# nmwsharp/diffusion-net

Hardware: NVIDIA H100
Metric: DiffusionNetBlock forward Mverts/sec at V=200k,K=128,C=128; 1/2/4/8 GPU (higher is better)
Workload: dtype f32

## Files before the change

### diffusion-net_b200/csrc/dn_tc.cu

```cuda
#include "dn_internal.h"
#include "dn_tc_ptx.cuh"
#include <cuda.h>
#include <cudaTypedefs.h>
#include <cuda_bf16.h>
#include <string.h>

namespace {

using namespace tc;

constexpr int KC = 16;
constexpr int TILE_M = 128;
constexpr int W_RING_BYTES = 128 * 1024;
constexpr int W_NST_MAX = 8;
constexpr int CHAIN_THREADS = 384;
constexpr int A_BOX_BYTES = 8 * TILE_M * 4;
constexpr int A_STAGE_BYTES = 2 * A_BOX_BYTES;
constexpr int A_NST_MAX = 8;
constexpr int SMEM_OPTIN = 232448;
constexpr int OUT_ROWS = 64;
constexpr int OUT_BOX_BYTES = 8 * OUT_ROWS * 4;

template <int MODE, int NMAX>
struct ChainRing {
  static constexpr int STAGE = KC * NMAX * (MODE == MODE_TF32X3 ? 8 : MODE == MODE_TF32 ? 4 : 2);
  static constexpr int NST_FULL = W_RING_BYTES / STAGE < W_NST_MAX ? W_RING_BYTES / STAGE : W_NST_MAX;
  static constexpr int STG = NMAX <= 128 && MODE != MODE_BF16 ? 2 * OUT_ROWS * NMAX * 4 : 0;
  static constexpr int BIAS = (NMAX <= 128 ? DN_MAX_LAYERS : 1) * NMAX * 4;
  static constexpr int bars(int nst, int anst) { return 8 * (2 * nst + 2 * anst + 2); }
  static constexpr int bytes(int nst, int anst) { return nst * STAGE + anst * A_STAGE_BYTES + STG + BIAS + bars(nst, anst); }
  static constexpr bool kFull = bytes(NST_FULL, A_NST_MAX) <= SMEM_OPTIN;
  static constexpr int NST = kFull ? NST_FULL : NST_FULL - 2;
  static constexpr int A_NST = kFull ? A_NST_MAX : A_NST_MAX - 1;
  static constexpr int BARS = bars(NST, A_NST);
  static constexpr int SMEM = bytes(NST, A_NST);
  static_assert(SMEM <= SMEM_OPTIN, "rows_chain_kernel: shared memory over the opt-in limit");
};

__host__ __device__ __forceinline__ int64_t stage_stride(int N) { return (int64_t)KC * N * 8; }
__host__ __device__ __forceinline__ int64_t packed_bytes(int K, int N) {
  return (((K + KC - 1) / KC) * stage_stride(N) + 255) / 256 * 256;
}

struct PackJob {
  const float* W;
  const float* W2;
  float* dst;
  int64_t ldw;
  int n_split, w_trans, K, N, blk0, fmt;
};
constexpr int kMaxPackJobs = 3 + DN_MAX_LAYERS;
struct PackJobs {
  PackJob j[kMaxPackJobs];
  int n;
  TcSpectral sp;
  int sp_blocks;
  int64_t sp_stride;
};

__device__ __forceinline__ void pack_store(float* dst, int fmt, int N, int k, int n, float w) {
  char* base = reinterpret_cast<char*>(dst) + (int64_t)(k / KC) * stage_stride(N);
  const int kk = k % KC;
  if (fmt == 2) {
    *reinterpret_cast<__nv_bfloat16*>(base + kmajor_off<MODE_BF16>(kk, n, N)) = __float2bfloat16_rn(w);
    return;
  }
  float hi, lo;
  split_tf32(w, hi, lo);
  char* q = base + kmajor_off<MODE_TF32>(tf32_k_slot(kk), n, N);
  *reinterpret_cast<float*>(q) = hi;
  *reinterpret_cast<float*>(q + (int64_t)KC * N * 4) = lo;
}

__global__ void pack_weights_kernel(const __grid_constant__ PackJobs jobs) {
  int n, k;
  float w;
  if (jobs.sp.partial && (int)blockIdx.x < jobs.sp_blocks * jobs.sp.n_meshes) {
    const PackJob& J = jobs.j[0];
    const int K = J.K, N = J.N;
    __shared__ float red[8][33];
    const int b = jobs.sp.n_meshes > 1 ? (int)blockIdx.x / jobs.sp_blocks : 0;
    const int e = threadIdx.x & 31, sl = threadIdx.x >> 5;
    const int idx = ((int)blockIdx.x - b * jobs.sp_blocks) * 32 + e;
    if (jobs.sp.plain) {
      if (sl != 0 || idx >= K * N) return;
      pack_store(J.dst + b * jobs.sp_stride, J.fmt, N, idx / N, idx % N, jobs.sp.partial[(int64_t)b * K * N + idx]);
      return;
    }
    const int p0 = jobs.sp.mesh_cta_begin ? jobs.sp.mesh_cta_begin[b] : 0;
// ... 10 lines not shown
    k = idx / N; n = idx % N;
    const float sum = pairwise_sum<8>(&red[0][e], 33);
    const float t = dn_clamp_time(jobs.sp.time[n]);
    w = dn_heat(jobs.sp.evals[(int64_t)b * K + k], t) * sum;
    pack_store(J.dst + b * jobs.sp_stride, J.fmt, N, k, n, w);
    if (jobs.sp.sum_out) jobs.sp.sum_out[(int64_t)b * K * N + idx] = sum;
    if (b == 0 && k == K - 1 && !jobs.sp.no_clamp_writeback) jobs.sp.time[n] = t;
    return;
  }
  int ji = 0;
#pragma unroll
  for (int i = 1; i < kMaxPackJobs; ++i)
    if (i < jobs.n && (int)blockIdx.x >= jobs.j[i].blk0) ji = i;
  const PackJob& J = jobs.j[ji];
  const int K = J.K, N = J.N;
  const int idx = ((int)blockIdx.x - J.blk0) * blockDim.x + threadIdx.x;
  if (idx >= K * N) return;
  n = idx / K; k = idx % K;
  if (J.w_trans) w = (J.W2 && k >= J.n_split) ? J.W2[(int64_t)(k - J.n_split) * J.ldw + n] : J.W[(int64_t)k * J.ldw + n];
  else if (J.W2 && n >= J.n_split) w = J.W2[(int64_t)(n - J.n_split) * J.ldw + k];
  else w = J.W[(int64_t)n * J.ldw + k];
  pack_store(J.dst, J.fmt, N, k, n, w);
}

struct HcLayer {
  const float* wpack;
  const float* bias;
  const float* emul;
  const float* relu_mask;
  const float* row_scale;
  const float* residual;
  int64_t ld_res;
  float res_scale;
  float* out;
  int64_t ld_out;
  int K, N, relu, sibling;
};

struct HcParams {
  CUtensorMap amap[DN_MAX_SRC];
  CUtensorMap omap[DN_MAX_LAYERS];
  CUtensorMap rmap[DN_MAX_LAYERS];
  DnRowsSrc src;
  HcLayer layer[DN_MAX_LAYERS];
  int n_layers;
  int64_t V;
  const int32_t* tile_group;
  int64_t group_stride;
  const float* head_w;
  const float* head_b;
  float* head_out;
  int64_t ld_head_out;
  int head_n;
};
static_assert(sizeof(HcParams) <= 4096, "HcParams must fit the 4 KiB kernel parameter space");

template <int MODE, int NMAX, bool WIDE>
__global__ void __launch_bounds__(CHAIN_THREADS, 1) rows_chain_kernel(const __grid_constant__ HcParams p) {
  constexpr bool kChain = NMAX <= 128;
  constexpr bool kStage = ChainRing<MODE, NMAX>::STG > 0;
  constexpr int NB = NMAX / 16;
  using Ring = ChainRing<MODE, NMAX>;
  constexpr int NST = Ring::NST, STAGE_BYTES = Ring::STAGE, A_NST = Ring::A_NST;
  extern __shared__ __align__(1024) uint8_t smem[];
  uint8_t* aring = smem + NST * STAGE_BYTES;
  uint8_t* stage_out = aring + A_NST * A_STAGE_BYTES;
  float* sbias = reinterpret_cast<float*>(stage_out + Ring::STG);
  uint64_t* bars = reinterpret_cast<uint64_t*>(stage_out + Ring::STG + Ring::BIAS);
  const uint32_t full = smem_u32(bars), empty = smem_u32(bars + NST);
  const uint32_t afull = smem_u32(bars + 2 * NST), aempty = smem_u32(bars + 2 * NST + A_NST);
  const uint32_t rfull = smem_u32(bars + 2 * NST + 2 * A_NST);
  const int warp = threadIdx.x >> 5, lane = threadIdx.x & 31;
  if (threadIdx.x == 0) {
    for (int i = 0; i < NST; ++i) { mbar_init(full + 8 * i, 1); mbar_init(empty + 8 * i, 8); }
    for (int i = 0; i < A_NST; ++i) { mbar_init(afull + 8 * i, 1); mbar_init(aempty + 8 * i, 8); }
    for (int i = 0; i < 2; ++i) mbar_init(rfull + 8 * i, 1);
    fence_barrier_init();
  }
  __syncthreads();
  const int L = p.n_layers;
  const int64_t ntiles = (p.V + TILE_M - 1) / TILE_M;

  if (warp >= 8) {
    setmaxnreg_dec<40>();
    if (warp == 9 && lane == 0) {
      const int K0 = p.layer[0].K, nst0 = (K0 + KC - 1) / KC;
      uint32_t s = 0, ph = 0;
      for (int64_t tile = blockIdx.x; tile < ntiles; tile += gridDim.x)
        for (int c = 0; c < nst0; ++c) {
          const int nbox = c * KC + 8 < K0 ? 2 : 1;
          mbar_wait(aempty + 8 * s, ph ^ 1);
          mbar_arrive_expect_tx(afull + 8 * s, (uint32_t)(nbox * A_BOX_BYTES));
          for (int h = 0; h < nbox; ++h) {
            int kc = c * KC + 8 * h, sidx = 0;
            while (sidx + 1 < p.src.nsrc && kc >= p.src.width[sidx]) { kc -= p.src.width[sidx]; ++sidx; }
            tma_tile_2d_g2s(smem_u32(aring + s * A_STAGE_BYTES + h * A_BOX_BYTES), &p.amap[sidx], kc,
                            (int)(tile * TILE_M), afull + 8 * s);
          }
          if (++s == A_NST) { s = 0; ph ^= 1; }
        }
    }
    if (warp == 8 && lane == 0) {
      uint32_t s = 0, ph = 0;
      for (int64_t tile = blockIdx.x; tile < ntiles; tile += gridDim.x)
        for (int l = 0; l < L; ++l) {
          const HcLayer& Lr = p.layer[l];
          const int nst = (Lr.K + KC - 1) / KC;
          const int64_t sstride = stage_stride(Lr.N);
          const uint32_t bytes = (uint32_t)(MODE == MODE_TF32X3 ? sstride : (MODE == MODE_TF32 ? sstride / 2 : sstride / 4));
          const char* w = reinterpret_cast<const char*>(Lr.wpack);
          if (l == 0 && p.tile_group) w += (int64_t)__ldg(p.tile_group + tile) * p.group_stride * 4;
          for (int c = 0; c < nst; ++c) {
            mbar_wait(empty + 8 * s, ph ^ 1);
            mbar_arrive_expect_tx(full + 8 * s, bytes);
            tma_bulk_g2s(smem_u32(smem + s * STAGE_BYTES), w + c * sstride, bytes, full + 8 * s);
            if (++s == NST) { s = 0; ph ^= 1; }
          }
        }
    }
    return;
  }

  setmaxnreg_inc<232>();
  for (int l = 0; l < L; ++l) {
    const HcLayer& Lr = p.layer[l];
    if (!Lr.bias) continue;
    for (int n = threadIdx.x; n < Lr.N; n += 256) sbias[l * NMAX + n] = __ldg(Lr.bias + n);
  }
  named_bar_sync(1, 256);
  const int g = lane >> 2, t = lane & 3;
  const int rloc = (warp >> 2) * 64 + (warp & 3) * 16 + g;
  const int wg = warp >> 2;
  const bool elected = (threadIdx.x & 127) == 0;
  auto stg_box = [&](int b) { return reinterpret_cast<float*>(stage_out) + (wg * NMAX + 8 * b) * OUT_ROWS; };
  float acc[NB * 8];
  float act[kChain ? NB * 8 : 1];
  uint32_t s = 0, ph = 0, as = 0, aph = 0, rph = 0;

  for (int64_t tile = blockIdx.x; tile < ntiles; tile += gridDim.x) {
    const int64_t r0 = tile * TILE_M + rloc, r1 = r0 + 8;
    const bool ok0 = r0 < p.V, ok1 = r1 < p.V;
    const int row0 = (int)(tile * TILE_M) + wg * OUT_ROWS;
    for (int l = 0; l < L; ++l) {
      const HcLayer& Lr = p.layer[l];
      const int N = WIDE ? NMAX : Lr.N, nb = N / 16;
      const int K = (WIDE && l > 0) ? NMAX : Lr.K, nst = (K + KC - 1) / KC;
      const uint32_t lbo = (uint32_t)N * 16;
      int prev = -1;
      if constexpr (kStage) {
        if (Lr.residual && elected) {
          bulk_wait_read<0>();
          if (row0 < p.V) {
            mbar_arrive_expect_tx(rfull + 8 * wg, (uint32_t)(Lr.N / 8 * OUT_BOX_BYTES));
            for (int b = 0; b < Lr.N / 8; ++b)
              tma_tile_2d_g2s(smem_u32(stg_box(b)), &p.rmap[l], 8 * b, row0, rfull + 8 * wg);
          } else {
            mbar_arrive(rfull + 8 * wg);
          }
        }
      }
      auto prefetch_rows = [&](const float* base, int64_t ld) {
#pragma unroll
        for (int h = 0; h < 2; ++h) {
          if (!(h ? ok1 : ok0)) continue;
          const char* row = reinterpret_cast<const char*>(base + (h ? r1 : r0) * ld);
          for (int b = 128 * t; b < N * 4; b += 512) prefetch_l2(row + b);
          if (t == 0) prefetch_l2(row + N * 4 - 4);
        }
      };
      if (!kStage && Lr.residual) prefetch_rows(Lr.residual, Lr.ld_res);
      if (Lr.emul) prefetch_rows(Lr.emul, N);
      if (Lr.relu_mask) prefetch_rows(Lr.relu_mask, N);
      auto stage = [&](int c, const float2* q, bool two) {
        mbar_wait(full + 8 * s, ph);
        constexpr int SLICES = MODE == MODE_BF16 ? 1 : 2;
        uint32_t ah[2][4], al[2][4];
        if constexpr (MODE == MODE_BF16) {
          const float x[8] = {q[0].x, q[0].y, q[1].x, q[1].y, q[2].x, q[2].y, q[3].x, q[3].y};
          frag_bf16(x, ah[0]);
        } else {
#pragma unroll
          for (int ks = 0; ks < 2; ++ks) {
            const float2 u = q[2 * ks], v = q[2 * ks + 1];
            const float x[4] = {u.x, v.x, u.y, v.y};
            frag_tf32(x, ah[ks], al[ks]);
          }
        }
        const uint32_t sb = smem_u32(smem + s * STAGE_BYTES);
        wgmma_fence();
#pragma unroll
        for (int ks = 0; ks < SLICES; ++ks) {
          if (ks == 1 && !two) break;
          const uint32_t acc0 = (c > 0 || ks > 0) ? 1u : 0u;
          const uint32_t base = sb + ks * 2 * lbo;
          if constexpr (WIDE) {
            mma_step<MODE, NMAX>(acc, ah[ks], al[ks], base, KC * N * 4, lbo, acc0);
          } else {
#pragma unroll
            for (int j = 0; j < NB; ++j) {
              if (j >= nb) break;
              mma_step<MODE, 16>(acc + 8 * j, ah[ks], al[ks], base + j * 256, KC * N * 4, lbo, acc0);
            }
          }
        }
        wgmma_commit();
        if constexpr (WIDE && MODE != MODE_BF16) {
          wgmma_wait<0>();
          if (lane == 0) mbar_arrive(empty + 8 * s);
        } else {
          wgmma_wait<1>();
          if (prev >= 0 && lane == 0) mbar_arrive(empty + 8 * prev);
          prev = (int)s;
        }
        if (++s == NST) { s = 0; ph ^= 1; }
      };

      if (l == 0) {
        for (int c = 0; c < nst; ++c) {
          const bool two = c * KC + 8 < K;
          mbar_wait(afull + 8 * as, aph);
          const float* a = reinterpret_cast<const float*>(aring + as * A_STAGE_BYTES) + rloc * 8 + 2 * t;
          float2 q[4];
          q[0] = *reinterpret_cast<const float2*>(a);
          q[1] = *reinterpret_cast<const float2*>(a + 64);
          q[2] = q[3] = make_float2(0.f, 0.f);
          if (two) {
            q[2] = *reinterpret_cast<const float2*>(a + A_BOX_BYTES / 4);
            q[3] = *reinterpret_cast<const float2*>(a + A_BOX_BYTES / 4 + 64);
          }
          stage(c, q, two);
          fence_proxy_async();
          __syncwarp();
          if (lane == 0) mbar_arrive(aempty + 8 * as);
          if (++as == A_NST) { as = 0; aph ^= 1; }
        }
      } else if constexpr (kChain) {
#pragma unroll
        for (int c = 0; c < NB; ++c) {
          if (c >= nst) break;
          const float2 q[4] = {make_float2(act[8 * c], act[8 * c + 1]), make_float2(act[8 * c + 2], act[8 * c + 3]),
                               make_float2(act[8 * c + 4], act[8 * c + 5]), make_float2(act[8 * c + 6], act[8 * c + 7])};
          stage(c, q, WIDE || c * KC + 8 < K);
        }
      }
      wgmma_wait<0>();
#pragma unroll
      for (int j = 0; j < NB; ++j) fence_acc8(acc + 8 * j);
      if (prev >= 0 && lane == 0) mbar_arrive(empty + 8 * prev);

      const bool last = l + 1 == L;
      const bool head = last && p.head_w != nullptr;
      const bool keep_act = !last && p.layer[l + 1].sibling;
      const float rs0 = (Lr.row_scale && ok0) ? __ldg(Lr.row_scale + r0) : 1.f;
      const float rs1 = (Lr.row_scale && ok1) ? __ldg(Lr.row_scale + r1) : 1.f;
      float hp0[kChain ? 1 : 8], hp1[kChain ? 1 : 8];
#pragma unroll
      for (int o = 0; o < (kChain ? 1 : 8); ++o) hp0[o] = hp1[o] = 0.f;
      if constexpr (kStage) {
        if (Lr.residual) {
          if (elected) mbar_wait(rfull + 8 * wg, rph);
          rph ^= 1;
          named_bar_sync(2 + wg, 128);
        } else if (Lr.out) {
          if (elected) bulk_wait_read<0>();
          named_bar_sync(2 + wg, 128);
        }
      }
      const int nb_epi = Lr.N / 16;
#pragma unroll
      for (int j = 0; j < NB; ++j) {
        if (j >= nb_epi) break;
#pragma unroll
        for (int h = 0; h < 2; ++h) {
          const int col = 16 * j + 8 * h + 2 * t;
          float* d = acc + 8 * j + 4 * h;
          float2 v0 = make_float2(d[0], d[1]), v1 = make_float2(d[2], d[3]);
          if (Lr.bias) {
            const float2 b = *reinterpret_cast<const float2*>(sbias + l * NMAX + col);
            const float b0 = b.x, b1 = b.y;
            v0.x += b0; v0.y += b1; v1.x += b0; v1.y += b1;
          }
          if (Lr.relu) {
            v0.x = fmaxf(v0.x, 0.f); v0.y = fmaxf(v0.y, 0.f); v1.x = fmaxf(v1.x, 0.f); v1.y = fmaxf(v1.y, 0.f);
          }
          if (Lr.emul) {
            if (ok0) { const float2 e = __ldg(reinterpret_cast<const float2*>(Lr.emul + r0 * N + col)); v0.x *= e.x; v0.y *= e.y; }
            if (ok1) { const float2 e = __ldg(reinterpret_cast<const float2*>(Lr.emul + r1 * N + col)); v1.x *= e.x; v1.y *= e.y; }
          }
          if (Lr.relu_mask) {
            if (ok0) {
              const float2 m = __ldg(reinterpret_cast<const float2*>(Lr.relu_mask + r0 * N + col));
              v0.x = m.x > 0.f ? v0.x : 0.f; v0.y = m.y > 0.f ? v0.y : 0.f;
            }
            if (ok1) {
              const float2 m = __ldg(reinterpret_cast<const float2*>(Lr.relu_mask + r1 * N + col));
              v1.x = m.x > 0.f ? v1.x : 0.f; v1.y = m.y > 0.f ? v1.y : 0.f;
            }
          }
          if (Lr.row_scale) { v0.x *= rs0; v0.y *= rs0; v1.x *= rs1; v1.y *= rs1; }
          if constexpr (kStage) {
            float* so = stg_box(2 * j + h) + ((warp & 3) * 16 + g) * 8 + 2 * t;
            if (Lr.residual) {
              const float2 ra = *reinterpret_cast<const float2*>(so), rb = *reinterpret_cast<const float2*>(so + 64);
              v0.x = fmaf(Lr.res_scale, ra.x, v0.x); v0.y = fmaf(Lr.res_scale, ra.y, v0.y);
              v1.x = fmaf(Lr.res_scale, rb.x, v1.x); v1.y = fmaf(Lr.res_scale, rb.y, v1.y);
            }
            if (Lr.out) {
              *reinterpret_cast<float2*>(so) = v0;
              *reinterpret_cast<float2*>(so + 64) = v1;
            }
          } else {
            if (Lr.residual) {
              if (ok0) {
                const float2 r = __ldg(reinterpret_cast<const float2*>(Lr.residual + r0 * Lr.ld_res + col));
                v0.x = fmaf(Lr.res_scale, r.x, v0.x); v0.y = fmaf(Lr.res_scale, r.y, v0.y);
              }
              if (ok1) {
                const float2 r = __ldg(reinterpret_cast<const float2*>(Lr.residual + r1 * Lr.ld_res + col));
                v1.x = fmaf(Lr.res_scale, r.x, v1.x); v1.y = fmaf(Lr.res_scale, r.y, v1.y);
              }
            }
            if (Lr.out) {
              if (ok0) *reinterpret_cast<float2*>(Lr.out + r0 * Lr.ld_out + col) = v0;
              if (ok1) *reinterpret_cast<float2*>(Lr.out + r1 * Lr.ld_out + col) = v1;
            }
          }
          if constexpr (kChain) {
            if (!keep_act) {
              act[8 * j + 4 * h] = v0.x; act[8 * j + 4 * h + 1] = v0.y;
              act[8 * j + 4 * h + 2] = v1.x; act[8 * j + 4 * h + 3] = v1.y;
            }
          }
          if (!kChain && head) {
#pragma unroll
            for (int o = 0; o < (kChain ? 1 : 8); ++o) {
              if (o >= p.head_n) break;
              const float2 w = __ldg(reinterpret_cast<const float2*>(p.head_w + (int64_t)o * N + col));
              hp0[o] = fmaf(w.y, v0.y, fmaf(w.x, v0.x, hp0[o]));
              hp1[o] = fmaf(w.y, v1.y, fmaf(w.x, v1.x, hp1[o]));
            }
          }
        }
      }
      if constexpr (kStage) {
        if (Lr.out || Lr.residual) {
          fence_proxy_async();
          named_bar_sync(2 + wg, 128);
          if (Lr.out && elected && row0 < p.V) {
            for (int b = 0; b < Lr.N / 8; ++b)
              tma_tile_2d_s2g(&p.omap[l], 8 * b, row0, smem_u32(stg_box(b)));
            bulk_commit();
            if (tile + gridDim.x >= ntiles) bulk_wait<0>();
          }
        }
      }
      if (head) {
        auto head_store = [&](int o, float a0, float a1) {
          a0 += __shfl_xor_sync(0xffffffffu, a0, 1);
          a0 += __shfl_xor_sync(0xffffffffu, a0, 2);
          a1 += __shfl_xor_sync(0xffffffffu, a1, 1);
          a1 += __shfl_xor_sync(0xffffffffu, a1, 2);
          const float b = p.head_b ? __ldg(p.head_b + o) : 0.f;
          if (t == 0 && ok0) p.head_out[r0 * p.ld_head_out + o] = a0 + b;
          if (t == 0 && ok1) p.head_out[r1 * p.ld_head_out + o] = a1 + b;
        };
        if constexpr (kChain) {
#pragma unroll 1
          for (int o = 0; o < p.head_n; ++o) {
            float a0 = 0.f, a1 = 0.f;
#pragma unroll
            for (int j = 0; j < NB; ++j) {
              if (j >= nb) break;
#pragma unroll
              for (int h = 0; h < 2; ++h) {
                const float* v = act + 8 * j + 4 * h;
                const float2 w = __ldg(reinterpret_cast<const float2*>(p.head_w + (int64_t)o * N + 16 * j + 8 * h + 2 * t));
                a0 = fmaf(w.y, v[1], fmaf(w.x, v[0], a0));
                a1 = fmaf(w.y, v[3], fmaf(w.x, v[2], a1));
              }
            }
            head_store(o, a0, a1);
          }
        } else {
#pragma unroll
          for (int o = 0; o < (kChain ? 1 : 8); ++o) {
            if (o >= p.head_n) break;
            head_store(o, hp0[o], hp1[o]);
          }
        }
      }
    }
  }
}

constexpr int TB_ROWS = 32;
constexpr int TB_NST = 3;
constexpr int TB_BOX = TB_ROWS * 8 * 4;
constexpr int TB_RAW_HALF = 16 * TB_BOX;
constexpr int TB_RAW = 2 * TB_RAW_HALF;
constexpr int TB_BIMG = TB_ROWS * 128 * 4;
constexpr int TB_BSTAGE = 2 * TB_BIMG;
constexpr int TB_THREADS = 288;
constexpr int TB_SUMS = 64 * 256 * 4;
constexpr int TB_SMEM = TB_NST * TB_RAW + 2 * TB_BSTAGE + TB_SUMS + 256;
constexpr int TB_FOLD = 128 / TB_ROWS;
static_assert(TB_SMEM <= 227 * 1024, "to_basis shared memory");

struct TcToBasisParams {
  CUtensorMap phi_map;
  CUtensorMap x_map;
  const float* mass;
  float* partial;
  int64_t V;
  int K, C;
  int64_t chunks_per_cta;
  int64_t ldp;
  const int32_t* cta_rows;
};

template <int MODE, int NBC>
__global__ void __launch_bounds__(TB_THREADS, 1) to_basis_kernel(const __grid_constant__ TcToBasisParams p) {
  extern __shared__ __align__(1024) uint8_t smem[];
  uint8_t* raw = smem;
  uint8_t* bimg = smem + TB_NST * TB_RAW;
  float* sums = reinterpret_cast<float*>(bimg + 2 * TB_BSTAGE);
  uint64_t* bars = reinterpret_cast<uint64_t*>(bimg + 2 * TB_BSTAGE + TB_SUMS);
  const uint32_t st_full = smem_u32(bars), st_empty = smem_u32(bars + TB_NST);
  const int warp = threadIdx.x >> 5, lane = threadIdx.x & 31;
  if (threadIdx.x == 0) {
    for (int i = 0; i < TB_NST; ++i) { mbar_init(st_full + 8 * i, 1); mbar_init(st_empty + 8 * i, 8); }
    fence_barrier_init();
// ... 99 lines not shown
#pragma unroll
    for (int ks = 0; ks < 4; ++ks) {
      const uint32_t acc0 = (fold > 0 || ks > 0) ? 1u : 0u;
      const uint32_t base = sb + ks * 2 * lbo;
      if constexpr (NBC == 8) {
        mma_step<MODE, 128>(acc, ah[ks], al[ks], base, TB_BIMG, lbo, acc0);
      } else {
#pragma unroll
        for (int j = 0; j < NBC; ++j) mma_step<MODE, 16>(acc + 8 * j, ah[ks], al[ks], base + j * 256, TB_BIMG, lbo, acc0);
      }
    }
    wgmma_commit();
  }
  wgmma_wait<0>();
#pragma unroll
  for (int j = 0; j < 8; ++j) fence_acc8(acc + 8 * j);
  if (nst > 0)
#pragma unroll
    for (int i = 0; i < 64; ++i) sum[256 * i] += acc[i];
  float* out = p.partial + (int64_t)blockIdx.x * K * p.ldp;
#pragma unroll
  for (int b = 0; b < 16; ++b) {
    const int col = 8 * b + 2 * t;
    if (col >= C) break;
    if (m0 < K) *reinterpret_cast<float2*>(out + (int64_t)m0 * p.ldp + col) = make_float2(sum[256 * (4 * b)], sum[256 * (4 * b + 1)]);
    if (m0 + 8 < K)
      *reinterpret_cast<float2*>(out + (int64_t)(m0 + 8) * p.ldp + col) = make_float2(sum[256 * (4 * b + 2)], sum[256 * (4 * b + 3)]);
  }
}

constexpr int kMaxDev = 64;
struct DevState { int queried, sms, sm90, tc_tried, tc; };
DevState g_dev[kMaxDev];

template <typename F>
bool set_smem(F* f, int bytes) {
  return cudaFuncSetAttribute(f, cudaFuncAttributeMaxDynamicSharedMemorySize, bytes) == cudaSuccess;
}
template <int MODE, int NBC0 = 1>
bool set_to_basis_smem() {
  if constexpr (NBC0 > 8) return true;
  else return set_smem(to_basis_kernel<MODE, NBC0>, TB_SMEM) && set_to_basis_smem<MODE, NBC0 + 1>();
}
template <int MODE, int NBC0 = 1>
void launch_to_basis(int nbc, int grid, const TcToBasisParams& p, cudaStream_t st) {
  if constexpr (NBC0 <= 8) {
    if (nbc == NBC0) to_basis_kernel<MODE, NBC0><<<grid, TB_THREADS, TB_SMEM, st>>>(p);
    else launch_to_basis<MODE, NBC0 + 1>(nbc, grid, p, st);
  }
}
template <int MODE>
bool set_chain_smem() {
  constexpr int s128 = ChainRing<MODE, 128>::SMEM, s256 = ChainRing<MODE, 256>::SMEM;
  return set_smem(rows_chain_kernel<MODE, 128, false>, s128) && set_smem(rows_chain_kernel<MODE, 128, true>, s128) &&
         set_smem(rows_chain_kernel<MODE, 256, false>, s256) && set_smem(rows_chain_kernel<MODE, 256, true>, s256);
}

PFN_cuTensorMapEncodeTiled_v12000 tensor_map_encoder() {
  static const PFN_cuTensorMapEncodeTiled_v12000 fn = [] {
    void* f = nullptr;
    cudaDriverEntryPointQueryResult q;
    if (cudaGetDriverEntryPointByVersion("cuTensorMapEncodeTiled", &f, 12000, cudaEnableDefault, &q) != cudaSuccess ||
        q != cudaDriverEntryPointSuccess) {
      cudaGetLastError();
      f = nullptr;
    }
    return reinterpret_cast<PFN_cuTensorMapEncodeTiled_v12000>(f);
  }();
  return fn;
}

}

bool encode_tensor_map_f32(CUtensorMap* m, const float* base, int64_t rows, int width, int64_t ld, int box_cols,
                           int box_rows, bool swizzle128) {
  const PFN_cuTensorMapEncodeTiled_v12000 encode = tensor_map_encoder();
  if (!encode) return false;
  const cuuint64_t dims[2] = {(cuuint64_t)width, (cuuint64_t)rows};
  const cuuint64_t strides[1] = {(cuuint64_t)ld * 4};
  const cuuint32_t box[2] = {(cuuint32_t)box_cols, (cuuint32_t)box_rows}, estr[2] = {1, 1};
  return encode(m, CU_TENSOR_MAP_DATA_TYPE_FLOAT32, 2, const_cast<float*>(base), dims, strides, box, estr,
                CU_TENSOR_MAP_INTERLEAVE_NONE, swizzle128 ? CU_TENSOR_MAP_SWIZZLE_128B : CU_TENSOR_MAP_SWIZZLE_NONE,
                CU_TENSOR_MAP_L2_PROMOTION_L2_256B, CU_TENSOR_MAP_FLOAT_OOB_FILL_NONE) == CUDA_SUCCESS;
}

static DevState* cur_dev_state() {
  int dev = 0;
  if (cudaGetDevice(&dev) != cudaSuccess || dev < 0 || dev >= kMaxDev) {
    cudaGetLastError();
    return nullptr;
  }
  DevState& d = g_dev[dev];
  if (!d.queried) {
    d.queried = 1;
    int major = 0, minor = 0;
    if (cudaDeviceGetAttribute(&d.sms, cudaDevAttrMultiProcessorCount, dev) != cudaSuccess ||
        cudaDeviceGetAttribute(&major, cudaDevAttrComputeCapabilityMajor, dev) != cudaSuccess ||
        cudaDeviceGetAttribute(&minor, cudaDevAttrComputeCapabilityMinor, dev) != cudaSuccess) {
      cudaGetLastError();
      major = 0;
    }
    if (d.sms < 1) d.sms = 1;
    d.sm90 = major == 9 && minor == 0;
  }
  return &d;
}

int dn_sm_count() {
// ... 41 lines not shown
    if (L.head_w && (!L.head_out || L.head_n < 1 || L.head_n > 8 || !aligned8(L.head_w))) return DN_ERR_UNSUPPORTED;
  }
  return DN_OK;
}

int tc_chain_plan(const DnRowsSrc& src, DnLayer* layers, int n_layers, int passes) {
  int fmt;
  if (passes == DN_PASSES_BF16 && chain_supported(src, layers, n_layers, true) == DN_OK) fmt = 2;
  else if (chain_supported(src, layers, n_layers, false) == DN_OK) fmt = 0;
  else return DN_ERR_UNSUPPORTED;
  for (int l = 0; l < n_layers; ++l) layers[l].pack_fmt = fmt;
  return fmt;
}

int64_t tc_chain_ws_bytes(const DnLayer* layers, int n_layers, int n_meshes) {
  int64_t b = (n_meshes - 1) * packed_bytes(layers[0].K, layers[0].N);
  for (int l = 0; l < n_layers; ++l) b += packed_bytes(layers[l].K, layers[l].N);
  return b;
}

int tc_pack_layers(DnLayer* layers, int n_layers, void* ws, int64_t ws_bytes, const TcSpectral* sp, cudaStream_t st) {
  if (n_layers < 1 || n_layers > kMaxPackJobs || (sp && sp->n_meshes < 1)) return DN_ERR_INVALID_ARGUMENT;
  if (tc_chain_ws_bytes(layers, n_layers, sp ? sp->n_meshes : 1) > ws_bytes || !ws) return DN_ERR_WORKSPACE;
  PackJobs jobs;
  memset(&jobs, 0, sizeof(jobs));
  jobs.n = n_layers;
  char* wp = static_cast<char*>(ws);
  int blocks = 0;
  for (int l = 0; l < n_layers; ++l) {
    DnLayer& L = layers[l];
    PackJob& J = jobs.j[l];
    J.W = L.W; J.W2 = L.W2; J.n_split = L.n_split; J.ldw = L.ldw; J.w_trans = L.w_trans; J.K = L.K; J.N = L.N;
    J.fmt = L.pack_fmt;
    J.dst = reinterpret_cast<float*>(wp);
    J.blk0 = blocks;
    L.prepacked = J.dst;
    if (l == 0 && sp) {
      jobs.sp = *sp;
      jobs.sp_blocks = (L.K * L.N + 31) / 32;
      jobs.sp_stride = packed_bytes(L.K, L.N) / 4;
      blocks += jobs.sp_blocks * sp->n_meshes;
      wp += packed_bytes(L.K, L.N) * sp->n_meshes;
      if (sp->tile_mesh) { L.tile_group = sp->tile_mesh; L.group_stride = jobs.sp_stride; }
    } else {
      blocks += (L.K * L.N + 255) / 256;
      wp += packed_bytes(L.K, L.N);
    }
  }
  pack_weights_kernel<<<blocks, 256, 0, st>>>(jobs);
  DN_LAUNCH_CHECK();
  return DN_OK;
}

template <int MODE>
static void launch_chain(const HcParams& p, int nmax, bool wide, int grid, cudaStream_t st) {
  constexpr int s128 = ChainRing<MODE, 128>::SMEM, s256 = ChainRing<MODE, 256>::SMEM;
  if (nmax <= 128) {
    if (wide) rows_chain_kernel<MODE, 128, true><<<grid, CHAIN_THREADS, s128, st>>>(p);
    else rows_chain_kernel<MODE, 128, false><<<grid, CHAIN_THREADS, s128, st>>>(p);
  } else {
    if (wide) rows_chain_kernel<MODE, 256, true><<<grid, CHAIN_THREADS, s256, st>>>(p);
    else rows_chain_kernel<MODE, 256, false><<<grid, CHAIN_THREADS, s256, st>>>(p);
  }
}

int tc_rows_chain(const DnRowsSrc& src, const DnLayer* layers_in, int n_layers, int64_t V, int passes, void* ws,
                  int64_t ws_bytes, cudaStream_t st) {
  if (V <= 0) return DN_OK;
  if (n_layers < 1 || n_layers > DN_MAX_LAYERS) return DN_ERR_INVALID_ARGUMENT;
  DnLayer layers[DN_MAX_LAYERS];
  bool packed = true;
  for (int l = 0; l < n_layers; ++l) {
    layers[l] = layers_in[l];
    packed = packed && layers[l].prepacked != nullptr;
  }
  if (!packed) {
    int rc = tc_pack_layers(layers, n_layers, ws, ws_bytes, nullptr, st);
    if (rc) return rc;
  }
  const bool bf16 = passes == DN_PASSES_BF16 && layers[0].pack_fmt == 2;
  if (passes == DN_PASSES_BF16 && !bf16) passes = 1;
  if (V >= (1ll << 31) - 256) return DN_ERR_UNSUPPORTED;
  HcParams p;
  memset(&p, 0, sizeof(p));
  p.src = src;
  p.n_layers = n_layers;
  p.V = V;
  p.tile_group = layers[0].tile_group;
  p.group_stride = layers[0].group_stride;
  for (int s = 0; s < src.nsrc; ++s)
    if (!encode_tensor_map_f32(&p.amap[s], src.ptr[s], V, src.width[s], src.ld[s], 8, TILE_M, false))
      return DN_ERR_UNSUPPORTED;
  int nmax = 0, nmin = 1 << 30;
  for (int l = 0; l < n_layers; ++l) {
    const DnLayer& L = layers[l];
    HcLayer& T = p.layer[l];
    T.wpack = L.prepacked; T.bias = L.bias; T.emul = L.emul; T.relu_mask = L.relu_mask_src; T.row_scale = L.row_scale;
    T.residual = L.residual; T.ld_res = L.ld_res; T.res_scale = L.res_scale; T.out = L.out; T.ld_out = L.ld_out;
    T.K = L.K; T.N = L.N; T.relu = L.relu; T.sibling = L.sibling;
    if (L.N > nmax) nmax = L.N;
    if (L.N < nmin) nmin = L.N;
  }
  if (nmax <= 128 && !bf16)
    for (int l = 0; l < n_layers; ++l) {
      const DnLayer& L = layers[l];
      if (L.out && !encode_tensor_map_f32(&p.omap[l], L.out, V, L.N, L.ld_out, 8, OUT_ROWS, false))
        return DN_ERR_UNSUPPORTED;
      if (L.residual && !encode_tensor_map_f32(&p.rmap[l], L.residual, V, L.N, L.ld_res, 8, OUT_ROWS, false))
        return DN_ERR_UNSUPPORTED;
    }
  const bool wide = nmin == nmax && (nmax == 128 || nmax == 256);
  const DnLayer& Ll = layers[n_layers - 1];
  p.head_w = Ll.head_w; p.head_b = Ll.head_b; p.head_out = Ll.head_out; p.ld_head_out = Ll.ld_head_out; p.head_n = Ll.head_n;
  const int64_t ntiles = (V + TILE_M - 1) / TILE_M;
  const int sms = dn_sm_count();
  const int grid = (int)(ntiles < sms ? ntiles : sms);
  if (bf16) launch_chain<MODE_BF16>(p, nmax, wide, grid, st);
  else if (passes == 3) launch_chain<MODE_TF32X3>(p, nmax, wide, grid, st);
  else launch_chain<MODE_TF32>(p, nmax, wide, grid, st);
  DN_LAUNCH_CHECK();
  return DN_OK;
}

int tc_to_basis_supported(int K, int C) {
  if (K % 4 || K < 4 || K > 128) return DN_ERR_UNSUPPORTED;
  if (C % 16 || C < 16 || C > 128) return DN_ERR_UNSUPPORTED;
  return DN_OK;
}

int tc_to_basis_partial(const float* values, const float* basis, const float* massvec, int64_t V, int K, int C,
                        float* partial, int* P_out, int passes, cudaStream_t st, int64_t ld_values, int64_t ldp,
                        const int32_t* cta_rows, int n_ctas) {
  if (tc_to_basis_supported(K, C) != DN_OK) return DN_ERR_UNSUPPORTED;
  if (ld_values <= 0) ld_values = C;
  if (ldp <= 0) ldp = C;
  if ((reinterpret_cast<uintptr_t>(values) & 15) || (reinterpret_cast<uintptr_t>(basis) & 15) || (ld_values % 4) ||
      (ldp % 2) || (reinterpret_cast<uintptr_t>(partial) & 7))
    return DN_ERR_UNSUPPORTED;
  if (V >= (1ll << 31) - 256) return DN_ERR_UNSUPPORTED;
  TcToBasisParams p;
  memset(&p, 0, sizeof(p));
  const int64_t rows = V > 0 ? V : 1;
  if (!encode_tensor_map_f32(&p.phi_map, basis, rows, K, K, 8, TB_ROWS, false) ||
      !encode_tensor_map_f32(&p.x_map, values, rows, C, ld_values, 8, TB_ROWS, false))
    return DN_ERR_UNSUPPORTED;
  p.mass = massvec; p.partial = partial;
  p.ldp = ldp; p.cta_rows = cta_rows;
  p.V = V; p.K = K; p.C = C; p.chunks_per_cta = 0;
  int grid;
  if (cta_rows) {
    if (n_ctas < 1) return DN_ERR_INVALID_ARGUMENT;
    grid = n_ctas;
  } else {
    const int64_t total_chunks = (V + KC - 1) / KC;
    grid = dn_sm_count();
    if (total_chunks < grid) grid = (int)(total_chunks > 0 ? total_chunks : 1);
    p.chunks_per_cta = (total_chunks + grid - 1) / grid;
    if (p.chunks_per_cta < 1) p.chunks_per_cta = 1;
    grid = (int)((total_chunks + p.chunks_per_cta - 1) / p.chunks_per_cta);
    if (grid < 1) grid = 1;
  }
  if (passes == 3) launch_to_basis<MODE_TF32X3>(C / 16, grid, p, st);
  else launch_to_basis<MODE_TF32>(C / 16, grid, p, st);
  DN_LAUNCH_CHECK();
  *P_out = grid;
  return DN_OK;
}
```

Measured before the change: 212.4.

## Skew warpgroup start in rows chain kernel to stagger weight-ring consumption

Adds a start-skew mbarrier so one consumer warpgroup waits until the other has consumed a configurable number of weight stages before starting its tile loop. The default skew is nonzero only for the TF32x3, N=128, wide variant, and an environment variable can override it. The aim is to desynchronize the two warpgroups so their wgmma bursts and epilogues interleave rather than contend simultaneously. The trade-off is extra startup latency, one more barrier in shared memory, and a risk of deadlock or phase errors if the skew interacts badly with ring depth.

```diff
diff --git a/diffusion-net_b200/csrc/dn_tc.cu b/diffusion-net_b200/csrc/dn_tc.cu
--- a/diffusion-net_b200/csrc/dn_tc.cu
+++ b/diffusion-net_b200/csrc/dn_tc.cu
@@ -3,6 +3,7 @@
 #include <cuda.h>
 #include <cudaTypedefs.h>
 #include <cuda_bf16.h>
+#include <stdlib.h>
 #include <string.h>
 
 namespace {
@@ -27,7 +28,7 @@
   static constexpr int NST_FULL = W_RING_BYTES / STAGE < W_NST_MAX ? W_RING_BYTES / STAGE : W_NST_MAX;
   static constexpr int STG = NMAX <= 128 && MODE != MODE_BF16 ? 2 * OUT_ROWS * NMAX * 4 : 0;
   static constexpr int BIAS = (NMAX <= 128 ? DN_MAX_LAYERS : 1) * NMAX * 4;
-  static constexpr int bars(int nst, int anst) { return 8 * (2 * nst + 2 * anst + 2); }
+  static constexpr int bars(int nst, int anst) { return 8 * (2 * nst + 2 * anst + 3); }
   static constexpr int bytes(int nst, int anst) { return nst * STAGE + anst * A_STAGE_BYTES + STG + BIAS + bars(nst, anst); }
   static constexpr bool kFull = bytes(NST_FULL, A_NST_MAX) <= SMEM_OPTIN;
   static constexpr int NST = kFull ? NST_FULL : NST_FULL - 2;
@@ -35,6 +36,7 @@
   static constexpr int BARS = bars(NST, A_NST);
   static constexpr int SMEM = bytes(NST, A_NST);
   static_assert(SMEM <= SMEM_OPTIN, "rows_chain_kernel: shared memory over the opt-in limit");
+  static constexpr int SKEW_MAX = NST < A_NST ? NST : A_NST;
 };
 
 __host__ __device__ __forceinline__ int64_t stage_stride(int N) { return (int64_t)KC * N * 8; }
@@ -151,6 +153,7 @@
   float* head_out;
   int64_t ld_head_out;
   int head_n;
+  int skew;
 };
 static_assert(sizeof(HcParams) <= 4096, "HcParams must fit the 4 KiB kernel parameter space");
 
@@ -169,11 +172,13 @@
   const uint32_t full = smem_u32(bars), empty = smem_u32(bars + NST);
   const uint32_t afull = smem_u32(bars + 2 * NST), aempty = smem_u32(bars + 2 * NST + A_NST);
   const uint32_t rfull = smem_u32(bars + 2 * NST + 2 * A_NST);
+  const uint32_t skew_bar = rfull + 16;
   const int warp = threadIdx.x >> 5, lane = threadIdx.x & 31;
   if (threadIdx.x == 0) {
     for (int i = 0; i < NST; ++i) { mbar_init(full + 8 * i, 1); mbar_init(empty + 8 * i, 8); }
     for (int i = 0; i < A_NST; ++i) { mbar_init(afull + 8 * i, 1); mbar_init(aempty + 8 * i, 8); }
     for (int i = 0; i < 2; ++i) mbar_init(rfull + 8 * i, 1);
+    mbar_init(skew_bar, 1);
     fence_barrier_init();
   }
   __syncthreads();
@@ -235,6 +240,10 @@
   float acc[NB * 8];
   float act[kChain ? NB * 8 : 1];
   uint32_t s = 0, ph = 0, as = 0, aph = 0, rph = 0;
+  if (p.skew > 0) {
+    if (elected) mbar_wait(skew_bar, wg ^ 1);
+    named_bar_sync(2 + wg, 128);
+  }
 
   for (int64_t tile = blockIdx.x; tile < ntiles; tile += gridDim.x) {
     const int64_t r0 = tile * TILE_M + rloc, r1 = r0 + 8;
@@ -311,6 +320,7 @@
           if (prev >= 0 && lane == 0) mbar_arrive(empty + 8 * prev);
           prev = (int)s;
         }
+        if (ph == 0 && (int)s + 1 == p.skew && threadIdx.x == 0) mbar_arrive(skew_bar);
         if (++s == NST) { s = 0; ph ^= 1; }
       };
 
@@ -830,15 +840,38 @@
   return DN_OK;
 }
 
+template <int MODE, int NMAX, bool WIDE>
+constexpr int kChainSkew = 0;
+template <>
+constexpr int kChainSkew<MODE_TF32X3, 128, true> = ChainRing<MODE_TF32X3, 128>::SKEW_MAX;
+
+static int chain_skew_env() {
+  static const int d = [] {
+    const char* e = getenv("DN_CHAIN_SKEW");
+    return e && *e ? atoi(e) : -1;
+  }();
+  return d;
+}
+
+template <int MODE, int NMAX, bool WIDE>
+static void launch_chain_kernel(HcParams& p, int grid, cudaStream_t st) {
+  using Ring = ChainRing<MODE, NMAX>;
+  int d = chain_skew_env() >= 0 ? chain_skew_env() : kChainSkew<MODE, NMAX, WIDE>;
+  if (d > Ring::SKEW_MAX) d = Ring::SKEW_MAX;
+  int tile_stages = 0;
+  for (int l = 0; l < p.n_layers; ++l) tile_stages += (p.layer[l].K + KC - 1) / KC;
+  p.skew = d < tile_stages ? d : tile_stages;
+  rows_chain_kernel<MODE, NMAX, WIDE><<<grid, CHAIN_THREADS, Ring::SMEM, st>>>(p);
+}
+
 template <int MODE>
-static void launch_chain(const HcParams& p, int nmax, bool wide, int grid, cudaStream_t st) {
-  constexpr int s128 = ChainRing<MODE, 128>::SMEM, s256 = ChainRing<MODE, 256>::SMEM;
+static void launch_chain(HcParams& p, int nmax, bool wide, int grid, cudaStream_t st) {
   if (nmax <= 128) {
-    if (wide) rows_chain_kernel<MODE, 128, true><<<grid, CHAIN_THREADS, s128, st>>>(p);
-    else rows_chain_kernel<MODE, 128, false><<<grid, CHAIN_THREADS, s128, st>>>(p);
+    if (wide) launch_chain_kernel<MODE, 128, true>(p, grid, st);
+    else launch_chain_kernel<MODE, 128, false>(p, grid, st);
   } else {
-    if (wide) rows_chain_kernel<MODE, 256, true><<<grid, CHAIN_THREADS, s256, st>>>(p);
-    else rows_chain_kernel<MODE, 256, false><<<grid, CHAIN_THREADS, s256, st>>>(p);
+    if (wide) launch_chain_kernel<MODE, 256, true>(p, grid, st);
+    else launch_chain_kernel<MODE, 256, false>(p, grid, st);
   }
 }
 
```

New measurement: 217.6, median of 6. 1.02x the previous value.

## Add three-consumer-warpgroup chain kernel variant with shared-memory activations

Applied to the files above, without the earlier changes.

Adds a variant of the fused MLP chain kernel with three consumer warpgroups, giving 192-row tiles instead of 128. Inter-layer activations stay in shared-memory staging rather than registers so register pressure fits 160 per thread. Residual loads are issued per warp in 16-row boxes, interleaved with the A-operand consumption. The weight and A rings shrink to fit shared memory, which may reduce pipelining depth, and the path is only selected for wide 128-channel multi-layer chains without siblings or tile groups.

```diff
diff --git a/diffusion-net_b200/csrc/dn_tc.cu b/diffusion-net_b200/csrc/dn_tc.cu
--- a/diffusion-net_b200/csrc/dn_tc.cu
+++ b/diffusion-net_b200/csrc/dn_tc.cu
@@ -10,31 +10,37 @@
 using namespace tc;
 
 constexpr int KC = 16;
-constexpr int TILE_M = 128;
 constexpr int W_RING_BYTES = 128 * 1024;
 constexpr int W_NST_MAX = 8;
-constexpr int CHAIN_THREADS = 384;
-constexpr int A_BOX_BYTES = 8 * TILE_M * 4;
-constexpr int A_STAGE_BYTES = 2 * A_BOX_BYTES;
 constexpr int A_NST_MAX = 8;
 constexpr int SMEM_OPTIN = 232448;
 constexpr int OUT_ROWS = 64;
 constexpr int OUT_BOX_BYTES = 8 * OUT_ROWS * 4;
-
-template <int MODE, int NMAX>
+constexpr int RES_ROWS = 16;
+
+template <int MODE, int NMAX, int CWG = 2>
 struct ChainRing {
+  static_assert(CWG == 2 || (CWG == 3 && NMAX == 128 && MODE != MODE_BF16), "rows_chain_kernel: unsupported variant");
+  static constexpr int TILE = 64 * CWG;
+  static constexpr int THREADS = 128 * CWG + 128;
+  static constexpr int A_BOX = 8 * TILE * 4;
+  static constexpr int A_STAGE = 2 * A_BOX;
   static constexpr int STAGE = KC * NMAX * (MODE == MODE_TF32X3 ? 8 : MODE == MODE_TF32 ? 4 : 2);
-  static constexpr int NST_FULL = W_RING_BYTES / STAGE < W_NST_MAX ? W_RING_BYTES / STAGE : W_NST_MAX;
-  static constexpr int STG = NMAX <= 128 && MODE != MODE_BF16 ? 2 * OUT_ROWS * NMAX * 4 : 0;
+  static constexpr int W_BYTES = CWG == 2 ? W_RING_BYTES : W_RING_BYTES / 2;
+  static constexpr int NST_FULL = W_BYTES / STAGE < W_NST_MAX ? W_BYTES / STAGE : W_NST_MAX;
+  static constexpr int A_NST_FULL = CWG == 2 ? A_NST_MAX : 5;
+  static constexpr int STG = NMAX <= 128 && MODE != MODE_BF16 ? CWG * OUT_ROWS * NMAX * 4 : 0;
   static constexpr int BIAS = (NMAX <= 128 ? DN_MAX_LAYERS : 1) * NMAX * 4;
-  static constexpr int bars(int nst, int anst) { return 8 * (2 * nst + 2 * anst + 2); }
-  static constexpr int bytes(int nst, int anst) { return nst * STAGE + anst * A_STAGE_BYTES + STG + BIAS + bars(nst, anst); }
-  static constexpr bool kFull = bytes(NST_FULL, A_NST_MAX) <= SMEM_OPTIN;
+  static constexpr int RBARS = CWG;
+  static constexpr int bars(int nst, int anst) { return 8 * (2 * nst + 2 * anst + RBARS); }
+  static constexpr int bytes(int nst, int anst) { return nst * STAGE + anst * A_STAGE + STG + BIAS + bars(nst, anst); }
+  static constexpr bool kFull = bytes(NST_FULL, A_NST_FULL) <= SMEM_OPTIN;
   static constexpr int NST = kFull ? NST_FULL : NST_FULL - 2;
-  static constexpr int A_NST = kFull ? A_NST_MAX : A_NST_MAX - 1;
+  static constexpr int A_NST = kFull ? A_NST_FULL : A_NST_FULL - 1;
   static constexpr int BARS = bars(NST, A_NST);
   static constexpr int SMEM = bytes(NST, A_NST);
   static_assert(SMEM <= SMEM_OPTIN, "rows_chain_kernel: shared memory over the opt-in limit");
+  static_assert(CWG == 2 || kFull, "rows_chain_kernel: the three-warpgroup rings are sized to fit");
 };
 
 __host__ __device__ __forceinline__ int64_t stage_stride(int N) { return (int64_t)KC * N * 8; }
@@ -154,13 +160,17 @@
 };
 static_assert(sizeof(HcParams) <= 4096, "HcParams must fit the 4 KiB kernel parameter space");
 
-template <int MODE, int NMAX, bool WIDE>
-__global__ void __launch_bounds__(CHAIN_THREADS, 1) rows_chain_kernel(const __grid_constant__ HcParams p) {
+template <int MODE, int NMAX, bool WIDE, int CWG = 2>
+__global__ void __launch_bounds__(ChainRing<MODE, NMAX, CWG>::THREADS, 1) rows_chain_kernel(const __grid_constant__ HcParams p) {
   constexpr bool kChain = NMAX <= 128;
-  constexpr bool kStage = ChainRing<MODE, NMAX>::STG > 0;
+  constexpr bool kStage = ChainRing<MODE, NMAX, CWG>::STG > 0;
+  constexpr bool kSmemAct = CWG == 3;
+  static_assert(!kSmemAct || (WIDE && kStage), "rows_chain_kernel: three consumer warpgroups need full-width staging");
   constexpr int NB = NMAX / 16;
-  using Ring = ChainRing<MODE, NMAX>;
+  using Ring = ChainRing<MODE, NMAX, CWG>;
   constexpr int NST = Ring::NST, STAGE_BYTES = Ring::STAGE, A_NST = Ring::A_NST;
+  constexpr int TILE = Ring::TILE, A_BOX_BYTES = Ring::A_BOX, A_STAGE_BYTES = Ring::A_STAGE;
+  constexpr int NCW = 4 * CWG;
   extern __shared__ __align__(1024) uint8_t smem[];
   uint8_t* aring = smem + NST * STAGE_BYTES;
   uint8_t* stage_out = aring + A_NST * A_STAGE_BYTES;
@@ -171,18 +181,18 @@
   const uint32_t rfull = smem_u32(bars + 2 * NST + 2 * A_NST);
   const int warp = threadIdx.x >> 5, lane = threadIdx.x & 31;
   if (threadIdx.x == 0) {
-    for (int i = 0; i < NST; ++i) { mbar_init(full + 8 * i, 1); mbar_init(empty + 8 * i, 8); }
-    for (int i = 0; i < A_NST; ++i) { mbar_init(afull + 8 * i, 1); mbar_init(aempty + 8 * i, 8); }
-    for (int i = 0; i < 2; ++i) mbar_init(rfull + 8 * i, 1);
+    for (int i = 0; i < NST; ++i) { mbar_init(full + 8 * i, 1); mbar_init(empty + 8 * i, NCW); }
+    for (int i = 0; i < A_NST; ++i) { mbar_init(afull + 8 * i, 1); mbar_init(aempty + 8 * i, NCW); }
+    for (int i = 0; i < Ring::RBARS; ++i) mbar_init(rfull + 8 * i, CWG == 2 ? 1 : 4);
     fence_barrier_init();
   }
   __syncthreads();
   const int L = p.n_layers;
-  const int64_t ntiles = (p.V + TILE_M - 1) / TILE_M;
-
-  if (warp >= 8) {
-    setmaxnreg_dec<40>();
-    if (warp == 9 && lane == 0) {
+  const int64_t ntiles = (p.V + TILE - 1) / TILE;
+
+  if (warp >= NCW) {
+    setmaxnreg_dec<CWG == 2 ? 40 : 24>();
+    if (warp == NCW + 1 && lane == 0) {
       const int K0 = p.layer[0].K, nst0 = (K0 + KC - 1) / KC;
       uint32_t s = 0, ph = 0;
       for (int64_t tile = blockIdx.x; tile < ntiles; tile += gridDim.x)
@@ -194,12 +204,12 @@
             int kc = c * KC + 8 * h, sidx = 0;
             while (sidx + 1 < p.src.nsrc && kc >= p.src.width[sidx]) { kc -= p.src.width[sidx]; ++sidx; }
             tma_tile_2d_g2s(smem_u32(aring + s * A_STAGE_BYTES + h * A_BOX_BYTES), &p.amap[sidx], kc,
-                            (int)(tile * TILE_M), afull + 8 * s);
+                            (int)(tile * TILE), afull + 8 * s);
           }
           if (++s == A_NST) { s = 0; ph ^= 1; }
         }
     }
-    if (warp == 8 && lane == 0) {
+    if (warp == NCW && lane == 0) {
       uint32_t s = 0, ph = 0;
       for (int64_t tile = blockIdx.x; tile < ntiles; tile += gridDim.x)
         for (int l = 0; l < L; ++l) {
@@ -220,33 +230,54 @@
     return;
   }
 
-  setmaxnreg_inc<232>();
+  setmaxnreg_inc<CWG == 2 ? 232 : 160>();
   for (int l = 0; l < L; ++l) {
     const HcLayer& Lr = p.layer[l];
     if (!Lr.bias) continue;
-    for (int n = threadIdx.x; n < Lr.N; n += 256) sbias[l * NMAX + n] = __ldg(Lr.bias + n);
-  }
-  named_bar_sync(1, 256);
+    for (int n = threadIdx.x; n < Lr.N; n += 128 * CWG) sbias[l * NMAX + n] = __ldg(Lr.bias + n);
+  }
+  named_bar_sync(1, 128 * CWG);
   const int g = lane >> 2, t = lane & 3;
   const int rloc = (warp >> 2) * 64 + (warp & 3) * 16 + g;
   const int wg = warp >> 2;
   const bool elected = (threadIdx.x & 127) == 0;
   auto stg_box = [&](int b) { return reinterpret_cast<float*>(stage_out) + (wg * NMAX + 8 * b) * OUT_ROWS; };
   float acc[NB * 8];
-  float act[kChain ? NB * 8 : 1];
+  float act[kChain && !kSmemAct ? NB * 8 : 1];
   uint32_t s = 0, ph = 0, as = 0, aph = 0, rph = 0;
 
   for (int64_t tile = blockIdx.x; tile < ntiles; tile += gridDim.x) {
-    const int64_t r0 = tile * TILE_M + rloc, r1 = r0 + 8;
+    const int64_t r0 = tile * TILE + rloc, r1 = r0 + 8;
     const bool ok0 = r0 < p.V, ok1 = r1 < p.V;
-    const int row0 = (int)(tile * TILE_M) + wg * OUT_ROWS;
+    const int row0 = (int)(tile * TILE) + wg * OUT_ROWS;
     for (int l = 0; l < L; ++l) {
       const HcLayer& Lr = p.layer[l];
       const int N = WIDE ? NMAX : Lr.N, nb = N / 16;
       const int K = (WIDE && l > 0) ? NMAX : Lr.K, nst = (K + KC - 1) / KC;
       const uint32_t lbo = (uint32_t)N * 16;
       int prev = -1;
-      if constexpr (kStage) {
+      const bool pred_stored = kSmemAct && p.layer[l > 0 ? l - 1 : L - 1].out != nullptr;
+      auto residual_load = [&](int c) {
+        fence_proxy_async();
+        __syncwarp();
+        if (lane == 0) {
+          const int wrow0 = row0 + (warp & 3) * RES_ROWS;
+          if (c == 0) {
+            if (wrow0 < p.V) mbar_arrive_expect_tx(rfull + 8 * wg, (uint32_t)(N / 8 * RES_ROWS * 32));
+            else mbar_arrive(rfull + 8 * wg);
+          }
+          if (wrow0 < p.V)
+            for (int h = 0; h < 2; ++h)
+              tma_tile_2d_g2s(smem_u32(stg_box(2 * c + h) + (warp & 3) * RES_ROWS * 8), &p.rmap[l], 16 * c + 8 * h,
+                              wrow0, rfull + 8 * wg);
+        }
+      };
+      if constexpr (kSmemAct) {
+        if (pred_stored && Lr.residual) {
+          if (elected) bulk_wait_read<0>();
+          named_bar_sync(2 + wg, 128);
+        }
+      } else if constexpr (kStage) {
         if (Lr.residual && elected) {
           bulk_wait_read<0>();
           if (row0 < p.V) {
@@ -332,6 +363,23 @@
           __syncwarp();
           if (lane == 0) mbar_arrive(aempty + 8 * as);
           if (++as == A_NST) { as = 0; aph ^= 1; }
+          if constexpr (kSmemAct) {
+            if (Lr.residual && c < nb) residual_load(c);
+          }
+        }
+        if constexpr (kSmemAct) {
+          if (Lr.residual)
+            for (int c = nst; c < nb; ++c) residual_load(c);
+        }
+      } else if constexpr (kSmemAct) {
+#pragma unroll
+        for (int c = 0; c < NB; ++c) {
+          const float* a = stg_box(2 * c) + ((warp & 3) * 16 + g) * 8 + 2 * t;
+          const float2 q[4] = {*reinterpret_cast<const float2*>(a), *reinterpret_cast<const float2*>(a + 64),
+                               *reinterpret_cast<const float2*>(a + 8 * OUT_ROWS),
+                               *reinterpret_cast<const float2*>(a + 8 * OUT_ROWS + 64)};
+          stage(c, q, true);
+          if (Lr.residual) residual_load(c);
         }
       } else if constexpr (kChain) {
 #pragma unroll
@@ -360,7 +408,7 @@
           if (elected) mbar_wait(rfull + 8 * wg, rph);
           rph ^= 1;
           named_bar_sync(2 + wg, 128);
-        } else if (Lr.out) {
+        } else if (kSmemAct ? pred_stored : Lr.out != nullptr) {
           if (elected) bulk_wait_read<0>();
           named_bar_sync(2 + wg, 128);
         }
@@ -404,7 +452,7 @@
               v0.x = fmaf(Lr.res_scale, ra.x, v0.x); v0.y = fmaf(Lr.res_scale, ra.y, v0.y);
               v1.x = fmaf(Lr.res_scale, rb.x, v1.x); v1.y = fmaf(Lr.res_scale, rb.y, v1.y);
             }
-            if (Lr.out) {
+            if (kSmemAct || Lr.out) {
               *reinterpret_cast<float2*>(so) = v0;
               *reinterpret_cast<float2*>(so + 64) = v1;
             }
@@ -424,7 +472,7 @@
               if (ok1) *reinterpret_cast<float2*>(Lr.out + r1 * Lr.ld_out + col) = v1;
             }
           }
-          if constexpr (kChain) {
+          if constexpr (kChain && !kSmemAct) {
             if (!keep_act) {
               act[8 * j + 4 * h] = v0.x; act[8 * j + 4 * h + 1] = v0.y;
               act[8 * j + 4 * h + 2] = v1.x; act[8 * j + 4 * h + 3] = v1.y;
@@ -442,7 +490,7 @@
         }
       }
       if constexpr (kStage) {
-        if (Lr.out || Lr.residual) {
+        if (Lr.out || (!kSmemAct && Lr.residual)) {
           fence_proxy_async();
           named_bar_sync(2 + wg, 128);
           if (Lr.out && elected && row0 < p.V) {
@@ -472,10 +520,17 @@
               if (j >= nb) break;
 #pragma unroll
               for (int h = 0; h < 2; ++h) {
-                const float* v = act + 8 * j + 4 * h;
                 const float2 w = __ldg(reinterpret_cast<const float2*>(p.head_w + (int64_t)o * N + 16 * j + 8 * h + 2 * t));
-                a0 = fmaf(w.y, v[1], fmaf(w.x, v[0], a0));
-                a1 = fmaf(w.y, v[3], fmaf(w.x, v[2], a1));
+                if constexpr (kSmemAct) {
+                  const float* so = stg_box(2 * j + h) + ((warp & 3) * 16 + g) * 8 + 2 * t;
+                  const float2 u0 = *reinterpret_cast<const float2*>(so), u1 = *reinterpret_cast<const float2*>(so + 64);
+                  a0 = fmaf(w.y, u0.y, fmaf(w.x, u0.x, a0));
+                  a1 = fmaf(w.y, u1.y, fmaf(w.x, u1.x, a1));
+                } else {
+                  const float* v = act + 8 * j + 4 * h;
+                  a0 = fmaf(w.y, v[1], fmaf(w.x, v[0], a0));
+                  a1 = fmaf(w.y, v[3], fmaf(w.x, v[2], a1));
+                }
               }
             }
             head_store(o, a0, a1);
@@ -681,8 +736,11 @@
 template <int MODE>
 bool set_chain_smem() {
   constexpr int s128 = ChainRing<MODE, 128>::SMEM, s256 = ChainRing<MODE, 256>::SMEM;
-  return set_smem(rows_chain_kernel<MODE, 128, false>, s128) && set_smem(rows_chain_kernel<MODE, 128, true>, s128) &&
-         set_smem(rows_chain_kernel<MODE, 256, false>, s256) && set_smem(rows_chain_kernel<MODE, 256, true>, s256);
+  bool ok = set_smem(rows_chain_kernel<MODE, 128, false>, s128) && set_smem(rows_chain_kernel<MODE, 128, true>, s128) &&
+            set_smem(rows_chain_kernel<MODE, 256, false>, s256) && set_smem(rows_chain_kernel<MODE, 256, true>, s256);
+  if constexpr (MODE != MODE_BF16)
+    ok = ok && set_smem(rows_chain_kernel<MODE, 128, true, 3>, ChainRing<MODE, 128, 3>::SMEM);
+  return ok;
 }
 
 PFN_cuTensorMapEncodeTiled_v12000 tensor_map_encoder() {
@@ -831,14 +889,22 @@
 }
 
 template <int MODE>
-static void launch_chain(const HcParams& p, int nmax, bool wide, int grid, cudaStream_t st) {
-  constexpr int s128 = ChainRing<MODE, 128>::SMEM, s256 = ChainRing<MODE, 256>::SMEM;
+static void launch_chain(const HcParams& p, int nmax, bool wide, int cwg, int grid, cudaStream_t st) {
+  using R128 = ChainRing<MODE, 128>;
+  using R256 = ChainRing<MODE, 256>;
+  if constexpr (MODE != MODE_BF16) {
+    if (cwg == 3) {
+      using R3 = ChainRing<MODE, 128, 3>;
+      rows_chain_kernel<MODE, 128, true, 3><<<grid, R3::THREADS, R3::SMEM, st>>>(p);
+      return;
+    }
+  }
   if (nmax <= 128) {
-    if (wide) rows_chain_kernel<MODE, 128, true><<<grid, CHAIN_THREADS, s128, st>>>(p);
-    else rows_chain_kernel<MODE, 128, false><<<grid, CHAIN_THREADS, s128, st>>>(p);
+    if (wide) rows_chain_kernel<MODE, 128, true><<<grid, R128::THREADS, R128::SMEM, st>>>(p);
+    else rows_chain_kernel<MODE, 128, false><<<grid, R128::THREADS, R128::SMEM, st>>>(p);
   } else {
-    if (wide) rows_chain_kernel<MODE, 256, true><<<grid, CHAIN_THREADS, s256, st>>>(p);
-    else rows_chain_kernel<MODE, 256, false><<<grid, CHAIN_THREADS, s256, st>>>(p);
+    if (wide) rows_chain_kernel<MODE, 256, true><<<grid, R256::THREADS, R256::SMEM, st>>>(p);
+    else rows_chain_kernel<MODE, 256, false><<<grid, R256::THREADS, R256::SMEM, st>>>(p);
   }
 }
 
@@ -866,10 +932,8 @@
   p.V = V;
   p.tile_group = layers[0].tile_group;
   p.group_stride = layers[0].group_stride;
-  for (int s = 0; s < src.nsrc; ++s)
-    if (!encode_tensor_map_f32(&p.amap[s], src.ptr[s], V, src.width[s], src.ld[s], 8, TILE_M, false))
-      return DN_ERR_UNSUPPORTED;
   int nmax = 0, nmin = 1 << 30;
+  bool sibling = false;
   for (int l = 0; l < n_layers; ++l) {
     const DnLayer& L = layers[l];
     HcLayer& T = p.layer[l];
@@ -878,24 +942,32 @@
     T.K = L.K; T.N = L.N; T.relu = L.relu; T.sibling = L.sibling;
     if (L.N > nmax) nmax = L.N;
     if (L.N < nmin) nmin = L.N;
-  }
+    sibling = sibling || L.sibling;
+  }
+  const bool wide = nmin == nmax && (nmax == 128 || nmax == 256);
+  const int sms = dn_sm_count();
+  const int cwg = !bf16 && wide && nmax == 128 && n_layers > 1 && !sibling && !p.tile_group && (V + 127) / 128 > sms
+                      ? 3 : 2;
+  const int tile_rows = 64 * cwg;
+  for (int s = 0; s < src.nsrc; ++s)
+    if (!encode_tensor_map_f32(&p.amap[s], src.ptr[s], V, src.width[s], src.ld[s], 8, tile_rows, false))
+      return DN_ERR_UNSUPPORTED;
   if (nmax <= 128 && !bf16)
     for (int l = 0; l < n_layers; ++l) {
       const DnLayer& L = layers[l];
       if (L.out && !encode_tensor_map_f32(&p.omap[l], L.out, V, L.N, L.ld_out, 8, OUT_ROWS, false))
         return DN_ERR_UNSUPPORTED;
-      if (L.residual && !encode_tensor_map_f32(&p.rmap[l], L.residual, V, L.N, L.ld_res, 8, OUT_ROWS, false))
+      if (L.residual &&
+          !encode_tensor_map_f32(&p.rmap[l], L.residual, V, L.N, L.ld_res, 8, cwg == 3 ? RES_ROWS : OUT_ROWS, false))
         return DN_ERR_UNSUPPORTED;
     }
-  const bool wide = nmin == nmax && (nmax == 128 || nmax == 256);
   const DnLayer& Ll = layers[n_layers - 1];
   p.head_w = Ll.head_w; p.head_b = Ll.head_b; p.head_out = Ll.head_out; p.ld_head_out = Ll.ld_head_out; p.head_n = Ll.head_n;
-  const int64_t ntiles = (V + TILE_M - 1) / TILE_M;
-  const int sms = dn_sm_count();
+  const int64_t ntiles = (V + tile_rows - 1) / tile_rows;
   const int grid = (int)(ntiles < sms ? ntiles : sms);
-  if (bf16) launch_chain<MODE_BF16>(p, nmax, wide, grid, st);
-  else if (passes == 3) launch_chain<MODE_TF32X3>(p, nmax, wide, grid, st);
-  else launch_chain<MODE_TF32>(p, nmax, wide, grid, st);
+  if (bf16) launch_chain<MODE_BF16>(p, nmax, wide, cwg, grid, st);
+  else if (passes == 3) launch_chain<MODE_TF32X3>(p, nmax, wide, cwg, grid, st);
+  else launch_chain<MODE_TF32>(p, nmax, wide, cwg, grid, st);
   DN_LAUNCH_CHECK();
   return DN_OK;
 }
```

Result: faster. 212.5 before, 227.8 after (median of 6 runs) (+7.2%).
